# Lucaskabela/UNAST

Measured on AMD Instinct MI355X. Metric: mel-frames/sec/node (train step, gen+disc) at B=32,T_mel=800; 1/2/4/8-GPU scaling, higher is better.
Workload: dtype bf16x3

## Files before the change

include/unast_hip.h:

```cpp
#ifndef UNAST_HIP_H
#define UNAST_HIP_H
#include <stdint.h>
#ifdef __cplusplus
extern "C" {
#endif

typedef struct ihipStream_t* hipStream_t;

const char* unast_last_error(void);
int unast_version(void);
const char* unast_arch(void);

int unast_gemm(int a_mode, int b_mode, int nsplit,
               const float* A, int lda, const float* B, int ldb, float* C, int ldc,
               int M, int N, int K, int kb_valid,
               int conv_T, int conv_ca, int conv_cb, int conv_shift,
               const float* bias, const float* R, int ldr, const float* G, int ldg, float gate_scale,
               float alpha, int beta, int act,
               float drop_p, unsigned int seed, unsigned int stream_id,
               int splitk, float* splitk_ws, int64_t splitk_ws_floats, float* rowsum_a, int tile_wn, int b_presplit,
               int out_split, double* colstats, hipStream_t stream);

int unast_attn_fwd(int nsplit, const float* Q, int ldq, const float* K, int ldk, const float* V, int ldv, float* O, int ldo,
                   float* LSE, const int* lens_k, int B, int H, int Tq, int Tk, int head_dim, int causal, float scale,
                   float drop_p, unsigned int seed, unsigned int stream_id, int qkv_split, hipStream_t stream);
int unast_attn_fwd_variant(int m32);
int unast_attn_bwd(int nsplit, const float* Q, int ldq, const float* K, int ldk, const float* V, int ldv, const float* O, int ldo,
                   const float* dO, int lddo, const float* LSE, float* delta_ws, float* dQ, int lddq, float* dK, int lddk,
                   float* dV, int lddv, const int* lens_k, int B, int H, int Tq, int Tk, int head_dim, int causal, float scale,
                   float drop_p, unsigned int seed, unsigned int stream_id, int fused, int qkv_split, const int* lens_q, hipStream_t stream);

int unast_layernorm_fwd(const float* z, const float* gamma, const float* beta, float* y, float* mean, float* rstd,
                        int rows, int C, float eps, hipStream_t stream);
int unast_layernorm_bwd(const float* dy, const float* z, const float* gamma, const float* mean, const float* rstd,
                        float* dz, float* dz_drop, float* dgamma, float* dbeta, float* ws, int64_t ws_floats, int rows, int C,
                        float drop_p, unsigned int seed, unsigned int stream_id, int finalize, hipStream_t stream);
int unast_layernorm_bwd_finalize(const float* ws, int64_t ws_floats, int rows, int C, float* dgamma, float* dbeta, hipStream_t stream);
int64_t unast_layernorm_bwd_ws_floats(int rows, int C);

int unast_colsum_f32(const float* x, int ldx, int rows, int C, float* sum, hipStream_t stream);
int unast_colsum_det(const float* x, int ldx, int rows, int C, float* sum, float* ws, int64_t ws_floats, hipStream_t stream);
int64_t unast_colsum_det_ws_floats(int rows, int C);

int unast_bn_fwd(const float* x, const float* gamma, const float* beta, float* y, float* mean, float* rstd,
                 float* running_mean, float* running_var, double* ws, int rows, int C,
                 float eps, float momentum, int act, float drop_p, unsigned int seed, unsigned int stream_id,
                 int have_sums, int64_t* num_batches_tracked, hipStream_t stream);
int unast_bn_eval_fwd(const float* x, const float* gamma, const float* beta, const float* running_mean,
                      const float* running_var, float* y, float* mean, float* rstd, int rows, int C, float eps, int act,
                      hipStream_t stream);
int unast_bn_bwd(float* dy_inout, const float* x, const float* mean, const float* rstd, const float* gamma, const float* beta,
                 float* dx, float* dgamma, float* dbeta, double* ws, int rows, int C, int act,
                 float drop_p, unsigned int seed, unsigned int stream_id, int ws_zeroed, hipStream_t stream);

int unast_embed_fwd(const int64_t* ids, const float* E, float* out, int rows, int T, int D, int shift_sos,
                    float drop_p, unsigned int seed, unsigned int stream_id, float noise_p, unsigned int noise_stream,
                    hipStream_t stream);
int unast_embed_bwd(const int64_t* ids, const float* dout, float* dE, int rows, int T, int D, int vocab, int shift_sos,
                    int padding_idx, float drop_p, unsigned int seed, unsigned int stream_id, float noise_p,
                    unsigned int noise_stream, hipStream_t stream);
int unast_embed_bwd_det(const int64_t* ids, const float* dout, float* dE, int rows, int T, int D, int vocab, int shift_sos,
                        int padding_idx, float drop_p, unsigned int seed, unsigned int stream_id, float noise_p,
                        unsigned int noise_stream, hipStream_t stream);

int unast_posenc_fwd(const float* x, const float* pe, float* y, int rows, int T, int D, float scale, float drop_p,
                     unsigned int seed, unsigned int stream_id, hipStream_t stream);
int unast_posenc_bwd(const float* dy, const float* gate, float* dx, int rows, int D, float scale, float drop_p,
                     unsigned int seed, unsigned int stream_id, hipStream_t stream);

int unast_rowmask(const float* x, float* y, int rows, int D, float p, unsigned int seed, unsigned int stream_id,
                  hipStream_t stream);
int unast_add_inplace(float* a, const float* b, int64_t n, hipStream_t stream);
int unast_sum2(float* dst, const float* a, const float* b, int64_t n, hipStream_t stream);
int unast_argmax_rows(const float* x, int ld, int rows, int cols, int64_t* out, hipStream_t stream);
int unast_mask_by_len(float* x, const int64_t* lens, int B, int T, int D, hipStream_t stream);
int unast_decode_linear(const float* X, int ldx, int64_t x_pos_stride, const float* W, int ldw, const float* bias, float* Y, int ldy, int M, int N, int K,
                        int act, float drop_p, unsigned int seed, unsigned int stream_id, const float* R, int ldr,
                        int prologue, const float* ln_gamma, const float* ln_beta, float ln_eps,
                        const int64_t* tokens, int ld_tok, const float* emb, const float* pe, float pro_scale,
                        float pro_drop1, unsigned int pro_stream1, float pro_drop2, unsigned int pro_stream2,
                        float* xn_out, int ld_xn,
                        float* cache, int ld_cache, int cache_rows, int split_col, const int64_t* pos, hipStream_t stream);
int unast_decode_attn(const float* Q, int ldq, const float* K, const float* V, int ldkv, int rows_per_seq, const int* lens,
// ... 110 lines not shown
```

unast_amd/config.py:

```python
import os

NSPLIT = 1 if os.environ.get("UNAST_PREC", "bf16x3").lower() in ("bf16", "1") else 3


def set_precision(name):
    global NSPLIT
    NSPLIT = {"bf16": 1, "bf16x3": 3}[name]


def precision_name():
    return "bf16" if NSPLIT == 1 else "bf16x3"


def snapshot():
    return tuple(sorted((k, v) for k, v in globals().items() if k.isupper()))


SIDE_STREAMS = os.environ.get("UNAST_SIDE_STREAMS", "1") != "0"

DECODE_GRAPH = os.environ.get("UNAST_DECODE_GRAPH", "1") != "0"

WGRAD_STREAM_MIN_TOKENS = int(os.environ.get("UNAST_WGRAD_MIN_TOKENS", "8192"))

DETERMINISTIC_SUMS = os.environ.get("UNAST_DETERMINISTIC_SUMS", "0") == "1"

CAPTURE_PRUNE = os.environ.get("UNAST_CAPTURE_PRUNE", "1") != "0"

WGRAD_GROUP = os.environ.get("UNAST_WGRAD_GROUP", "1") != "0"

ATTN_FUSED_BWD = os.environ.get("UNAST_ATTN_FUSED_BWD", "1") != "0"
ATTN_BWD_TERMS = int(os.environ.get("UNAST_ATTN_BWD_TERMS", "3"))

DGRAD_TRANSPOSED = os.environ.get("UNAST_DGRAD_T", "0") == "1"

PANEL_MIN_ROWS = int(os.environ.get("UNAST_PANEL_MIN_ROWS", "16384"))
PANEL_ROWS = int(os.environ.get("UNAST_PANEL_ROWS", "1128"))

NATIVE_COMM = os.environ.get("UNAST_NATIVE_COMM", "1") != "0"

ENC_SKIP_PAD_GRADS = os.environ.get("UNAST_ENC_SKIP_PAD_GRADS", "0") == "1"

STREAM_JITTER = int(os.environ.get("UNAST_STREAM_JITTER", "0"))
STREAM_JITTER_SEED = int(os.environ.get("UNAST_STREAM_JITTER_SEED", "0"))

DEBUG_WORKSPACES = os.environ.get("UNAST_DEBUG_WORKSPACES", "0") == "1"

JOINT_GEN = os.environ.get("UNAST_JOINT_GEN", "1") != "0"
```

unast_amd/csrc/attention.hip:

```cpp
#include "common.h"
#include <stdlib.h>
#include <type_traits>

#define HD 64
#define ALD 64
__device__ __forceinline__ int img_off(int row, int col) { return row * (ALD * 2) + ((((col >> 3) ^ (row & 6))) << 4) + ((col & 7) << 1); }
#define LOG2E 1.4426950408889634f
#define LN2 0.6931471805599453f
#define NEG_BIG (-1.0e30f)

struct AttnParams {
    const float* Q; const float* K; const float* V; int ldq, ldk, ldv;
    float* O; int ldo;
    float* LSE;
    const float* dO; int lddo;
    const float* Delta;
    float* dK; float* dV; int lddk, lddv;
    const int* lens_k;
    const int* lens_q;
    int B, H, Tq, Tk, causal;
    float scale;
    uint32_t drop_thresh; float drop_scale; uint32_t seed, stream;
    int qkv_split;
    int order;
// ... 507 lines not shown
                    }
                }
            lsum += rs;
        };
#ifndef KO_SOFTMAX
        if (interior) softmax_tile(std::false_type{}); else softmax_tile(std::true_type{});
#endif
#pragma unroll
        for (int t2 = 0; t2 < 2; ++t2) {
            bf16x8_t vfh[2][2], vfl[2][2];
#pragma unroll
            for (int v = 0; v < 2; ++v)
#pragma unroll
                for (int dt = 0; dt < 2; ++dt) {
                    vfh[v][dt] = vtr_frag32(sV[0], 32 * t2 + 16 * v, 32 * dt, lane);
                    vfl[v][dt] = (PARTS == 2) ? vtr_frag32(sV[PARTS - 1], 32 * t2 + 16 * v, 32 * dt, lane) : vfh[v][dt];
                }
            bf16x8_t ph[2], pl[2];
#pragma unroll
            for (int v = 0; v < 2; ++v)
                split8<NSPLIT>(make_float4(s[t2][8 * v], s[t2][8 * v + 1], s[t2][8 * v + 2], s[t2][8 * v + 3]),
                               make_float4(s[t2][8 * v + 4], s[t2][8 * v + 5], s[t2][8 * v + 6], s[t2][8 * v + 7]), ph[v], pl[v]);
            asm volatile("" : "+v"(vfh[0][0]), "+v"(vfh[0][1]), "+v"(vfh[1][0]), "+v"(vfh[1][1]));
            if (PARTS == 2) asm volatile("" : "+v"(vfl[0][0]), "+v"(vfl[0][1]), "+v"(vfl[1][0]), "+v"(vfl[1][1]));
#pragma unroll
            for (int v = 0; v < 2; ++v)
#pragma unroll
                for (int dt = 0; dt < 2; ++dt) {
#ifdef KO_PVMFMA
                    o[dt][2 * t2 + v] += __builtin_bit_cast(f32x4, vfh[v][dt])[0] + __builtin_bit_cast(f32x4, vfl[v][dt])[1] + __builtin_bit_cast(f32x4, ph[v])[0] + __builtin_bit_cast(f32x4, pl[v])[1];
#else
                    o[dt] = mma3_32<NSPLIT>(vfh[v][dt], vfl[v][dt], ph[v], pl[v], o[dt]);
#endif
                }
        }
        }
#ifndef KO_BARRIER
        __syncthreads();
#endif
    }
    const float ltot = half_sum(lsum);
    if (qok) {
        const float f = ltot > 0.f ? p.drop_scale / ltot : 0.f;
        float* dst = p.O + ((size_t)b * p.Tq + q) * p.ldo + h * HD + 4 * hi;
#pragma unroll
        for (int dt = 0; dt < 2; ++dt)
#pragma unroll
            for (int i4 = 0; i4 < 4; ++i4)
                *reinterpret_cast<float4*>(dst + 32 * dt + 8 * i4) = make_float4(o[dt][4 * i4] * f, o[dt][4 * i4 + 1] * f, o[dt][4 * i4 + 2] * f, o[dt][4 * i4 + 3] * f);
        if (hi == 0) p.LSE[((size_t)b * p.H + h) * p.Tq + q] = (m + log2f(ltot)) * LN2;
    }
}

template <int NSPLIT, int FUSE_DQ, int PLO>
__global__ __launch_bounds__(256, 2) void attn_dkv_kernel(const AttnParams p) {
    constexpr int PARTS = (NSPLIT == 3) ? 2 : 1;
    constexpr int SPARTS = PLO ? PARTS : 1;
    constexpr int IMG = 32 * ALD * 2;
    constexpr int IMG128 = 128 * ALD * 2;
    __shared__ __attribute__((aligned(16))) unsigned char smem[2 * PARTS * IMG + (FUSE_DQ ? (PARTS + SPARTS) * IMG128 : 0)];
    unsigned char* sQ[2] = {smem, smem + (PARTS - 1) * IMG};
    unsigned char* sD[2] = {smem + PARTS * IMG, smem + PARTS * IMG + (PARTS - 1) * IMG};
    unsigned char* const fbase = smem + 2 * PARTS * IMG;
    unsigned char* sKs[2] = {fbase, fbase + (PARTS - 1) * IMG128};
    unsigned char* sS[2] = {fbase + PARTS * IMG128, fbase + PARTS * IMG128 + (SPARTS - 1) * IMG128};

    const int t = threadIdx.x, lane = t & 63, wave = t >> 6, l15 = lane & 15, g = lane >> 4;
    int bx, bh;
    if (!xcd_remap((p.Tk + 127) / 128, p.B * p.H, bx, bh, p.order)) return;
    const int h = bh % p.H, b = bh / p.H;
    const int kblk = bx * 128;
    const int k0 = kblk + wave * 32;
    const int klen = p.lens_k ? min(p.Tk, p.lens_k[b]) : p.Tk;
    const bool wave_live = __builtin_amdgcn_readfirstlane((int)(k0 < klen)) != 0;
    const int kk_live = min(4, (max(klen - kblk, 0) + 31) >> 5);
    const float sc = p.scale * LOG2E;
    const float* Qb = p.Q + (size_t)b * p.Tq * p.ldq + h * HD;
    const float* Kb = p.K + (size_t)b * p.Tk * p.ldk + h * HD;
    const float* Vb = p.V + (size_t)b * p.Tk * p.ldv + h * HD;
    const float* dOb = p.dO + (size_t)b * p.Tq * p.lddo + h * HD;
    const float* lseb = p.LSE + ((size_t)b * p.H + h) * p.Tq;
    const float* delb = p.Delta + ((size_t)b * p.H + h) * p.Tq;

    const bool split_in = p.qkv_split != 0;
    bf16x8_t kf[2][2][PARTS], vf[2][2][PARTS];
#pragma unroll
    for (int ks = 0; ks < 2; ++ks) {
        const int key = k0 + 16 * ks + l15;
        const bool ok = key < p.Tk;
#pragma unroll
        for (int kst = 0; kst < 2; ++kst) {
            bf16x8_t hi, lo;
            if (!FUSE_DQ) {
                load_frag8<NSPLIT>(Kb + (size_t)key * p.ldk + 32 * kst + 8 * g, ok, split_in, 1.f, hi, lo);
                kf[ks][kst][0] = hi; if (PARTS == 2) kf[ks][kst][PARTS - 1] = lo;
            }
            load_frag8<NSPLIT>(Vb + (size_t)key * p.ldv + 32 * kst + 8 * g, ok, split_in, 1.f, hi, lo);
            vf[ks][kst][0] = hi; if (PARTS == 2) vf[ks][kst][PARTS - 1] = lo;
        }
    }
    f32x4 dk[4][2], dv[4][2];
#pragma unroll
    for (int dt = 0; dt < 4; ++dt)
#pragma unroll
        for (int ks = 0; ks < 2; ++ks) { dk[dt][ks] = (f32x4){0.f, 0.f, 0.f, 0.f}; dv[dt][ks] = dk[dt][ks]; }

    const uint32_t rbase = rng_stream_base(p.seed, p.stream);
    const bool block_live = kblk < klen;
    const int qt_begin = p.causal ? (kblk / 32) : 0;
    const int qlen = p.lens_q ? min(p.Tq, max(p.lens_q[b], 0)) : p.Tq;
    const int qt_end = block_live ? (qlen + 31) / 32 : qt_begin;
    float4 rq[2], rd[2];
    float rl = 0.f, rl_cur = 0.f;
    const float* const stat_src = (lane < 32) ? lseb : delb;
    const float stat_mul = (lane < 32) ? LOG2E : 1.f;
    auto stat_load = [&](int qtile) {
        rl = stat_src[min(qtile * 32 + (lane & 31), p.Tq - 1)];
    };
    if (FUSE_DQ && qt_begin < qt_end) {
        float4 rk8[8];
        tile_load<128>(Kb + (size_t)kblk * p.ldk, p.ldk, min(128, p.Tk - kblk), rk8, t);
        tile_store<128, NSPLIT>(rk8, sKs[0], sKs[PARTS - 1], t, split_in);
    }
    if (qt_begin < qt_end) {
        tile_load<32>(Qb + (size_t)qt_begin * 32 * p.ldq, p.ldq, min(32, p.Tq - qt_begin * 32), rq, t);
        tile_load<32>(dOb + (size_t)qt_begin * 32 * p.lddo, p.lddo, min(32, p.Tq - qt_begin * 32), rd, t);
        stat_load(qt_begin);
    }
    auto dq_phase = [&](int qtile, int buf) {
        f32x4 dq[2] = {(f32x4){0.f, 0.f, 0.f, 0.f}, (f32x4){0.f, 0.f, 0.f, 0.f}};
#pragma unroll
        for (int kk = 0; kk < 4; ++kk) {
            if (kk >= kk_live) break;
            const bf16x8_t bh = tr_frag(sKs[0], 32 * kk, 16 * wave, l15, g);
            const bf16x8_t bl = (PARTS == 2) ? tr_frag(sKs[PARTS - 1], 32 * kk, 16 * wave, l15, g) : bh;
#pragma unroll
            for (int qs = 0; qs < 2; ++qs) {
                const bf16x8_t ah = tr_frag(sS[0], 32 * kk, 32 * buf + 16 * qs, l15, g);
                if (SPARTS == 2) {
                    const bf16x8_t al = tr_frag(sS[SPARTS - 1], 32 * kk, 32 * buf + 16 * qs, l15, g);
                    dq[qs] = mma3<NSPLIT>(ah, al, bh, bl, dq[qs]);
                } else {
                    dq[qs] = mma2_a<NSPLIT>(ah, bh, bl, dq[qs]);
                }
            }
        }
        float* dqb = p.O + (size_t)b * p.Tq * p.ldo + h * HD + 16 * wave + l15;
#pragma unroll
        for (int qs = 0; qs < 2; ++qs)
#pragma unroll
            for (int r = 0; r < 4; ++r) {
                const int q = qtile * 32 + 16 * qs + 4 * g + r;
                if (q < p.Tq) unsafeAtomicAdd(dqb + (size_t)q * p.ldo, dq[qs][r] * p.scale);
            }
    };
    for (int qt = qt_begin; qt < qt_end; ++qt) {
        tile_store<32, NSPLIT>(rq, sQ[0], sQ[PARTS - 1], t, split_in);
        tile_store<32, NSPLIT>(rd, sD[0], sD[PARTS - 1], t, split_in);
        rl_cur = rl * stat_mul;
        const uint32_t rk_cur = p.drop_thresh ? pcg_hash((uint32_t)(((size_t)b * p.H + h) * p.Tq + qt * 32 + (lane & 31)) + rbase) : 0u;
        __syncthreads();
        if (FUSE_DQ && qt > qt_begin) dq_phase(qt - 1, (qt - 1) & 1);
        if (qt + 1 < qt_end) {
            const int qr = (qt + 1) * 32;
            tile_load<32>(Qb + (size_t)qr * p.ldq, p.ldq, min(32, p.Tq - qr), rq, t);
            tile_load<32>(dOb + (size_t)qr * p.lddo, p.lddo, min(32, p.Tq - qr), rd, t);
            stat_load(qt + 1);
        }
        if (wave_live) {
        f32x4 s[2][2], dp[2][2];
#pragma unroll
        for (int qs = 0; qs < 2; ++qs)
#pragma unroll
            for (int ks = 0; ks < 2; ++ks) { s[qs][ks] = (f32x4){0.f, 0.f, 0.f, 0.f}; dp[qs][ks] = s[qs][ks]; }
#pragma unroll
        for (int qs = 0; qs < 2; ++qs)
#pragma unroll
            for (int kst = 0; kst < 2; ++kst) {
                const bf16x8_t qh = row_frag(sQ[0], 16 * qs, kst, l15, g);
                const bf16x8_t ql = (PARTS == 2) ? row_frag(sQ[PARTS - 1], 16 * qs, kst, l15, g) : qh;
                const bf16x8_t dh = row_frag(sD[0], 16 * qs, kst, l15, g);
                const bf16x8_t dl = (PARTS == 2) ? row_frag(sD[PARTS - 1], 16 * qs, kst, l15, g) : dh;
#pragma unroll
                for (int ks = 0; ks < 2; ++ks) {
                    if (FUSE_DQ) {
                        const bf16x8_t kh = row_frag(sKs[0], wave * 32 + 16 * ks, kst, l15, g);
                        const bf16x8_t kl = (PARTS == 2) ? row_frag(sKs[PARTS - 1], wave * 32 + 16 * ks, kst, l15, g) : kh;
                        s[qs][ks] = mma3<NSPLIT>(qh, ql, kh, kl, s[qs][ks]);
                    } else {
                        s[qs][ks] = mma3<NSPLIT>(qh, ql, kf[ks][kst][0], kf[ks][kst][PARTS - 1], s[qs][ks]);
                    }
                    dp[qs][ks] = mma3<NSPLIT>(dh, dl, vf[ks][kst][0], vf[ks][kst][PARTS - 1], dp[qs][ks]);
                }
            }
        const bool interior = (qt * 32 + 32 <= p.Tq) && (k0 + 32 <= klen) && (!p.causal || k0 + 31 <= qt * 32);
        auto pointwise = [&](auto masked_tag) {
            constexpr bool MASKED = decltype(masked_tag)::value;
            const int par = l15 & 1;
            const uint32_t sh16 = par ? 0u : 16u, thr_hi = p.drop_thresh << 16;
#pragma unroll
            for (int qs = 0; qs < 2; ++qs) {
                float l2[4], de[4];
#pragma unroll
                for (int r = 0; r < 4; ++r) {
                    l2[r] = __shfl(rl_cur, 16 * qs + 4 * g + r, 64);
                    de[r] = __shfl(rl_cur, 32 + 16 * qs + 4 * g + r, 64);
                }
                uint32_t rkm[2] = {0u, 0u};
                if (p.drop_thresh) {
#pragma unroll
                    for (int j = 0; j < 2; ++j) rkm[j] = (uint32_t)__shfl((int)rk_cur, 16 * qs + 4 * g + 2 * par + j, 64);
                }
#pragma unroll
                for (int ks = 0; ks < 2; ++ks) {
                    const int key = k0 + 16 * ks + l15;
                    uint32_t hh[4] = {0u, 0u, 0u, 0u};
                    if (p.drop_thresh) {
#pragma unroll
                        for (int j = 0; j < 2; ++j) {
                            const uint32_t hm = rng_pair(rkm[j], (uint32_t)key);
                            hh[j] = (uint32_t)__builtin_amdgcn_mov_dpp((int)hm, 0xA0, 0xF, 0xF, true);
// ... 11 lines not shown
                        float pd = pv, dpe = dp[qs][ks][r];
                        if (p.drop_thresh) {
                            const bool keep = (hh[r] << sh16) >= thr_hi;
                            pd = keep ? pv : 0.f;
                            dpe = keep ? dpe : 0.f;
                        }
                        s[qs][ks][r] = pd;
                        dp[qs][ks][r] = pv * __builtin_fmaf(dpe, p.drop_scale, -de[r]);
                    }
                }
            }
        };
        if (interior) pointwise(std::false_type{}); else pointwise(std::true_type{});
        bf16x8_t pf[2][SPARTS], sf[2][SPARTS];
#pragma unroll
        for (int ks = 0; ks < 2; ++ks) {
            bf16x8_t hi, lo;
            pack_acc<(SPARTS == 2 ? NSPLIT : 1)>(s[0][ks], s[1][ks], hi, lo);
            pf[ks][0] = hi; if (SPARTS == 2) pf[ks][SPARTS - 1] = lo;
            pack_acc<(SPARTS == 2 ? NSPLIT : 1)>(dp[0][ks], dp[1][ks], hi, lo);
            sf[ks][0] = hi; if (SPARTS == 2) sf[ks][SPARTS - 1] = lo;
            if (FUSE_DQ) {
                const int row = wave * 32 + 16 * ks + l15, col = 32 * (qt & 1) + 4 * g;
                const u32x4 hw = __builtin_bit_cast(u32x4, hi), lw = __builtin_bit_cast(u32x4, lo);
                *reinterpret_cast<u32x2*>(sS[0] + img_off(row, col)) = (u32x2){hw[0], hw[1]};
                *reinterpret_cast<u32x2*>(sS[0] + img_off(row, col + 16)) = (u32x2){hw[2], hw[3]};
                if (SPARTS == 2) {
                    *reinterpret_cast<u32x2*>(sS[SPARTS - 1] + img_off(row, col)) = (u32x2){lw[0], lw[1]};
                    *reinterpret_cast<u32x2*>(sS[SPARTS - 1] + img_off(row, col + 16)) = (u32x2){lw[2], lw[3]};
                }
            }
        }
#pragma unroll
        for (int dt = 0; dt < 4; ++dt) {
            const bf16x8_t doh = tr_frag(sD[0], 0, 16 * dt, l15, g);
            const bf16x8_t dol = (PARTS == 2) ? tr_frag(sD[PARTS - 1], 0, 16 * dt, l15, g) : doh;
            const bf16x8_t qh = tr_frag(sQ[0], 0, 16 * dt, l15, g);
            const bf16x8_t ql = (PARTS == 2) ? tr_frag(sQ[PARTS - 1], 0, 16 * dt, l15, g) : qh;
#pragma unroll
            for (int ks = 0; ks < 2; ++ks) {
                if (SPARTS == 2) {
                    dv[dt][ks] = mma3<NSPLIT>(doh, dol, pf[ks][0], pf[ks][SPARTS - 1], dv[dt][ks]);
                    dk[dt][ks] = mma3<NSPLIT>(qh, ql, sf[ks][0], sf[ks][SPARTS - 1], dk[dt][ks]);
                } else {
                    dv[dt][ks] = mma2_b<NSPLIT>(doh, dol, pf[ks][0], dv[dt][ks]);
                    dk[dt][ks] = mma2_b<NSPLIT>(qh, ql, sf[ks][0], dk[dt][ks]);
                }
            }
        }
        }
        __syncthreads();
    }
    if (FUSE_DQ && qt_begin < qt_end) dq_phase(qt_end - 1, (qt_end - 1) & 1);
#pragma unroll
    for (int ks = 0; ks < 2; ++ks) {
        const int key = k0 + 16 * ks + l15;
        if (key >= p.Tk) continue;
        float* dkp = p.dK + ((size_t)b * p.Tk + key) * p.lddk + h * HD + 4 * g;
        float* dvp = p.dV + ((size_t)b * p.Tk + key) * p.lddv + h * HD + 4 * g;
#pragma unroll
        for (int dt = 0; dt < 4; ++dt) {
            *reinterpret_cast<float4*>(dkp + 16 * dt) = make_float4(dk[dt][ks][0] * p.scale, dk[dt][ks][1] * p.scale, dk[dt][ks][2] * p.scale, dk[dt][ks][3] * p.scale);
            *reinterpret_cast<float4*>(dvp + 16 * dt) = make_float4(dv[dt][ks][0] * p.drop_scale, dv[dt][ks][1] * p.drop_scale, dv[dt][ks][2] * p.drop_scale, dv[dt][ks][3] * p.drop_scale);
        }
    }
}

__global__ __launch_bounds__(256) void attn_delta_kernel(const float* __restrict__ dO, int lddo, const float* __restrict__ O, int ldo,
                                                         float* __restrict__ delta, int rows, int Tq, int H, float* __restrict__ zero_dq, int lddq,
                                                         int do_split) {
    const int lane = threadIdx.x & 63;
    const int row = blockIdx.x * 4 + (threadIdx.x >> 6);
    if (row >= rows) return;
    const int b = row / Tq, q = row - b * Tq;
    for (int h0 = 0; h0 < H; h0 += 4) {
        const int h = h0 + (lane >> 4);
        float s = 0.f;
        if (h < H) {
            const int c = h * HD + (lane & 15) * 4;
            float4 a = *reinterpret_cast<const float4*>(dO + (size_t)row * lddo + c);
            if (do_split) {
                const uint32_t h0 = __float_as_uint(a.x), h1 = __float_as_uint(a.y), l0 = __float_as_uint(a.z), l1 = __float_as_uint(a.w);
                a.x = __uint_as_float(h0 << 16) + __uint_as_float(l0 << 16);
                a.y = __uint_as_float(h0 & 0xFFFF0000u) + __uint_as_float(l0 & 0xFFFF0000u);
                a.z = __uint_as_float(h1 << 16) + __uint_as_float(l1 << 16);
                a.w = __uint_as_float(h1 & 0xFFFF0000u) + __uint_as_float(l1 & 0xFFFF0000u);
            }
            float4 o = *reinterpret_cast<const float4*>(O + (size_t)row * ldo + c);
            s = (a.x * o.x + a.y * o.y) + (a.z * o.z + a.w * o.w);
            if (zero_dq) *reinterpret_cast<float4*>(zero_dq + (size_t)row * lddq + c) = make_float4(0.f, 0.f, 0.f, 0.f);
        }
        s += __shfl_xor(s, 1, 64); s += __shfl_xor(s, 2, 64); s += __shfl_xor(s, 4, 64); s += __shfl_xor(s, 8, 64);
        if (h < H && (lane & 15) == 0) delta[((size_t)b * H + h) * Tq + q] = s;
    }
}

static bool al16(const void* p) { return (((uintptr_t)p) & 15) == 0; }

static int fill_common(AttnParams& p, const float* Q, int ldq, const float* K, int ldk, const float* V, int ldv, const int* lens_k,
                       int B, int H, int Tq, int Tk, int head_dim, int causal, float scale, float drop_p, unsigned seed, unsigned stream_id, int qkv_split) {
    UNAST_REQUIRE(Q && K && V, "unast_attn: null Q/K/V");
    UNAST_REQUIRE(head_dim == HD, "unast_attn: this build supports head_dim=%d only (got %d)", HD, head_dim);
    UNAST_REQUIRE(B > 0 && H > 0 && Tq > 0 && Tk > 0, "unast_attn: bad dims");
    UNAST_REQUIRE(al16(Q) && al16(K) && al16(V) && (ldq & 3) == 0 && (ldk & 3) == 0 && (ldv & 3) == 0, "unast_attn: Q/K/V must be 16-byte aligned with ld%%4==0");
    UNAST_REQUIRE(!causal || Tq == Tk, "unast_attn: causal masking requires Tq == Tk");
    p.Q = Q; p.K = K; p.V = V; p.ldq = ldq; p.ldk = ldk; p.ldv = ldv; p.lens_k = lens_k;
    p.B = B; p.H = H; p.Tq = Tq; p.Tk = Tk; p.causal = causal; p.scale = scale;
    p.drop_thresh = drop_threshold(drop_p); p.drop_scale = drop_p > 0.f ? 1.f / (1.f - drop_p) : 1.f; p.seed = seed; p.stream = stream_id;
    p.qkv_split = qkv_split;
    static const int forced = [] { const char* e = getenv("UNAST_ATTN_ORDER"); return e ? atoi(e) : -1; }();
    p.order = forced >= 0 ? forced : (causal ? 1 : 0);
    p.lens_q = nullptr;
    p.O = nullptr; p.LSE = nullptr; p.dO = nullptr; p.Delta = nullptr; p.dK = nullptr; p.dV = nullptr; p.ldo = p.lddo = p.lddk = p.lddv = 0;
    return UNAST_OK;
}

static int g_attn_fwd_m32 = [] { const char* e = getenv("UNAST_ATTN_FWD_M32"); return (e && e[0] == '0') ? 0 : 1; }();
extern "C" int unast_attn_fwd_variant(int m32) {
    const int old = g_attn_fwd_m32;
    if (m32 >= 0) g_attn_fwd_m32 = m32 ? 1 : 0;
    return old;
}

extern "C" int unast_attn_fwd(int nsplit, const float* Q, int ldq, const float* K, int ldk, const float* V, int ldv, float* O, int ldo,
                              float* LSE, const int* lens_k, int B, int H, int Tq, int Tk, int head_dim, int causal, float scale,
                              float drop_p, unsigned int seed, unsigned int stream_id, int qkv_split, hipStream_t stream) {
    AttnParams p;
    int rc = fill_common(p, Q, ldq, K, ldk, V, ldv, lens_k, B, H, Tq, Tk, head_dim, causal, scale, drop_p, seed, stream_id, qkv_split);
    if (rc) return rc;
    UNAST_REQUIRE(O && LSE && al16(O) && (ldo & 3) == 0, "unast_attn_fwd: bad output");
    UNAST_REQUIRE(nsplit == 1 || nsplit == 3, "unast_attn_fwd: nsplit must be 1 or 3");
    p.O = O; p.ldo = ldo; p.LSE = LSE;
    static const bool q16 = [] { const char* e = getenv("UNAST_ATTN_FWD_Q16"); return e && e[0] == '1'; }();
    dim3 grid(xcd_grid((Tq + 127) / 128, B * H));
    if (g_attn_fwd_m32 && !q16) {
        if (nsplit == 3) hipLaunchKernelGGL((attn_fwd32_kernel<3>), grid, dim3(256), 0, stream, p);
        else             hipLaunchKernelGGL((attn_fwd32_kernel<1>), grid, dim3(256), 0, stream, p);
        return unast_check_launch("unast_attn_fwd");
    }
    if (nsplit == 3) if (q16) hipLaunchKernelGGL((attn_q_kernel<3, 0, 1>), grid, dim3(512), 0, stream, p); else hipLaunchKernelGGL((attn_q_kernel<3, 0, 2>), grid, dim3(256), 0, stream, p);
    else             if (q16) hipLaunchKernelGGL((attn_q_kernel<1, 0, 1>), grid, dim3(512), 0, stream, p); else hipLaunchKernelGGL((attn_q_kernel<1, 0, 2>), grid, dim3(256), 0, stream, p);
    return unast_check_launch("unast_attn_fwd");
}

extern "C" int unast_attn_bwd(int nsplit, const float* Q, int ldq, const float* K, int ldk, const float* V, int ldv, const float* O, int ldo,
                              const float* dO, int lddo, const float* LSE, float* delta_ws, float* dQ, int lddq, float* dK, int lddk,
                              float* dV, int lddv, const int* lens_k, int B, int H, int Tq, int Tk, int head_dim, int causal, float scale,
                              float drop_p, unsigned int seed, unsigned int stream_id, int fused, int qkv_split, const int* lens_q, hipStream_t stream) {
    AttnParams p;
    int rc = fill_common(p, Q, ldq, K, ldk, V, ldv, lens_k, B, H, Tq, Tk, head_dim, causal, scale, drop_p, seed, stream_id, qkv_split);
    if (rc) return rc;
    UNAST_REQUIRE(O && dO && LSE && delta_ws && dQ && dK && dV, "unast_attn_bwd: null pointer");
    UNAST_REQUIRE(!lens_q || fused, "unast_attn_bwd: lens_q is served by the one-pass backward (fused = 1)");
    p.lens_q = lens_q;
    UNAST_REQUIRE(al16(O) && al16(dO) && al16(dQ) && al16(dK) && al16(dV) && ((ldo | lddo | lddq | lddk | lddv) & 3) == 0,
                  "unast_attn_bwd: operands must be 16-byte aligned with ld%%4==0");
    UNAST_REQUIRE(nsplit == 1 || nsplit == 3, "unast_attn_bwd: nsplit must be 1 or 3");
    const int rows = B * Tq;
    hipLaunchKernelGGL(attn_delta_kernel, dim3((rows + 3) / 4), dim3(256), 0, stream, dO, lddo, O, ldo, delta_ws, rows, Tq, H, fused ? dQ : nullptr, lddq, qkv_split);
    p.dO = dO; p.lddo = lddo; p.LSE = const_cast<float*>(LSE); p.Delta = delta_ws;
    p.O = dQ; p.ldo = lddq; p.dK = dK; p.dV = dV; p.lddk = lddk; p.lddv = lddv;
    dim3 gq(xcd_grid((Tq + 127) / 128, B * H)), gk(xcd_grid((Tk + 127) / 128, B * H));
    if (fused) {
        if (nsplit == 3) { if (fused == 1) hipLaunchKernelGGL((attn_dkv_kernel<3, 1, 1>), gk, dim3(256), 0, stream, p); else hipLaunchKernelGGL((attn_dkv_kernel<3, 1, 0>), gk, dim3(256), 0, stream, p); }
        else             hipLaunchKernelGGL((attn_dkv_kernel<1, 1, 1>), gk, dim3(256), 0, stream, p);
    } else if (nsplit == 3) {
        hipLaunchKernelGGL((attn_q_kernel<3, 1, 2>), gq, dim3(256), 0, stream, p);
        hipLaunchKernelGGL((attn_dkv_kernel<3, 0, 1>), gk, dim3(256), 0, stream, p);
    } else {
        hipLaunchKernelGGL((attn_q_kernel<1, 1, 2>), gq, dim3(256), 0, stream, p);
        hipLaunchKernelGGL((attn_dkv_kernel<1, 0, 1>), gk, dim3(256), 0, stream, p);
    }
    return unast_check_launch("unast_attn_bwd");
}

UNAST_DEFINE_RNG_EPOCH_SETTER(attention)
```

unast_amd/ops.py:

```python
import os as _os

import torch

from . import config
from ._lib import lib, check

OP_KC, OP_KC_CONV, OP_RC, OP_RC_CONV_DGRAD, OP_RC_CONV_WGRAD = 0, 1, 2, 3, 4


def _p(t):
    return None if t is None else t.data_ptr()


_raw_stream = getattr(torch._C, "_cuda_getCurrentRawStream", None)


def _stream():
    if _raw_stream is not None:
        return _raw_stream(torch.cuda.current_device())
    return torch.cuda.current_stream().cuda_stream


_F32 = torch.float32
_LN_WS = {}


def deterministic_sums():
    return bool(config.DETERMINISTIC_SUMS)


def _f32(t, name):
    if t is None:
        return
    if not (t.is_cuda and t.dtype == torch.float32):
        raise TypeError("%s must be a float32 CUDA tensor (got %s on %s)" % (name, t.dtype, t.device))


_WEIGHT_SPANS = []


def register_weight_span(base_ptr, nbytes, split_ptr, transposed_lookup=None, planes_lookup=None):
    _WEIGHT_SPANS[:] = [s for s in _WEIGHT_SPANS if s[0] != base_ptr]
    _WEIGHT_SPANS.append((base_ptr, nbytes, split_ptr, transposed_lookup, planes_lookup))


def unregister_weight_span(base_ptr):
    _WEIGHT_SPANS[:] = [s for s in _WEIGHT_SPANS if s[0] != base_ptr]


def _weight_planes(W, transposed=False):
    ptr = W.data_ptr()
    for base, nbytes, split, _, lookup in _WEIGHT_SPANS:
        if lookup is not None and base <= ptr < base + nbytes:
            return lookup(W, transposed)
    return None


# ... 321 lines not shown
    if _PANEL_TRACE:
        print("panel_gemm M=%d N=%d K=%d lda=%d ldc=%d bias=%s R=%s G=%s act=%d drop=%.2f split=%d ln=%s bits=%s rows=%d" % (
            M, N, K, A.stride(0), C.stride(0), bias is not None, R is not None, G is not None, act, drop_p, out_split, ln is not None,
            None if gate_bits is None else gate_bits.numel(), rows_per_wg), flush=True)
    check(lib().unast_panel_gemm(_p(A), A.stride(0), wplanes[0], wplanes[1], _p(C), C.stride(0), M, N, K, _p(bias), _p(R),
                                 R.stride(0) if R is not None else 0, _p(G), G.stride(0) if G is not None else 0, gate_scale, act,
                                 drop_p, seed & 0xFFFFFFFF, stream_id, int(out_split), _p(g), _p(b), _p(Y), ldy, _p(mean), _p(rstd), eps,
                                 _p(gate_bits), rows_per_wg, _stream()), "unast_panel_gemm")
    if _PANEL_TRACE:
        torch.cuda.synchronize()
    return C


def conv_fwd(x3d, Wp, bias, out, pad_left, colstats=None):
    B, T, Cin = x3d.shape
    Cout = Wp.shape[0]
    gemm(OP_KC_CONV, OP_KC, x3d, x3d.stride(1), Wp, 5 * Cin, out, out.stride(1), B * T, Cout, 5 * Cin,
         conv=(T, Cin, 0, pad_left), bias=bias, colstats=colstats)
    return out


def conv_dgrad(dy3d, Wp, dx, pad_left, beta=0):
    B, T, Cout = dy3d.shape
    Cin = Wp.shape[2]
    gemm(OP_KC_CONV, OP_RC_CONV_DGRAD, dy3d, dy3d.stride(1), Wp, 4, dx, dx.stride(1), B * T, Cin, 5 * Cout,
         conv=(T, Cout, Cout, 4 - pad_left), beta=beta)
    return dx


def conv_wgrad(dy3d, x3d, dWp, pad_left, db=None):
    B, T, Cout = dy3d.shape
    Cin = x3d.shape[2]
    sk = _splitk_for(Cout, 5 * Cin, B * T)
    if db is not None and deterministic_sums() and dy3d.is_contiguous():
        def both():
            gemm(OP_RC, OP_RC_CONV_WGRAD, dy3d, dy3d.stride(1), x3d, x3d.stride(1), dWp, 5 * Cin, Cout, 5 * Cin, B * T,
                 conv=(T, 0, Cin, pad_left), beta=1, splitk=sk)
            colsum(dy3d.view(B * T, Cout), db)
        _on_wgrad_stream(both, B * T, dWp.data_ptr(), dy3d, x3d)
        return dWp
    _on_wgrad_stream(lambda: gemm(OP_RC, OP_RC_CONV_WGRAD, dy3d, dy3d.stride(1), x3d, x3d.stride(1), dWp, 5 * Cin, Cout, 5 * Cin, B * T,
                                  conv=(T, 0, Cin, pad_left), beta=1, splitk=sk, rowsum_a=db), B * T, dWp.data_ptr(), dy3d, x3d)
    return dWp


def attn_fwd(Q, K, V, O, LSE, lens_k, B, H, Tq, Tk, causal, drop_p=0.0, seed=0, stream_id=0, nsplit=None, qkv_split=False):
    check(lib().unast_attn_fwd(nsplit or config.NSPLIT, _p(Q), Q.stride(0), _p(K), K.stride(0), _p(V), V.stride(0), _p(O), O.stride(0),
                               _p(LSE), _p(lens_k), B, H, Tq, Tk, 64, int(causal), 0.125, drop_p, seed & 0xFFFFFFFF, stream_id,
                               int(qkv_split), _stream()), "unast_attn_fwd")


def attn_bwd(Q, K, V, O, dO, LSE, delta_ws, dQ, dK, dV, lens_k, B, H, Tq, Tk, causal, drop_p=0.0, seed=0, stream_id=0, nsplit=None, qkv_split=False, lens_q=None):
    fused = config.ATTN_FUSED_BWD and not deterministic_sums()
    check(lib().unast_attn_bwd(nsplit or config.NSPLIT, _p(Q), Q.stride(0), _p(K), K.stride(0), _p(V), V.stride(0), _p(O), O.stride(0),
                               _p(dO), dO.stride(0), _p(LSE), _p(delta_ws), _p(dQ), dQ.stride(0), _p(dK), dK.stride(0), _p(dV),
                               dV.stride(0), _p(lens_k), B, H, Tq, Tk, 64, int(causal), 0.125, drop_p, seed & 0xFFFFFFFF, stream_id,
                               (2 if config.ATTN_BWD_TERMS == 2 else 1) if fused else 0, int(qkv_split),
                               _p(lens_q) if fused else None, _stream()), "unast_attn_bwd")


def layernorm_fwd(z, gamma, beta, y, mean, rstd, eps=1e-5):
    rows, C = z.shape
    check(lib().unast_layernorm_fwd(_p(z), _p(gamma), _p(beta), _p(y), _p(mean), _p(rstd), rows, C, eps, _stream()), "unast_layernorm_fwd")


def layernorm_bwd(dy, z, gamma, mean, rstd, dz, dz_drop=None, dgamma=None, dbeta=None, drop_p=0.0, seed=0, stream_id=0):
    rows, C = z.shape
    ws, ws_n = None, 0
    if dgamma is not None:
        ws_n = _LN_WS.get((rows, C))
        if ws_n is None:
            ws_n = _LN_WS[(rows, C)] = lib().unast_layernorm_bwd_ws_floats(rows, C)
        ws = torch.empty(ws_n, dtype=torch.float32, device=z.device)
    check(lib().unast_layernorm_bwd(_p(dy), _p(z), _p(gamma), _p(mean), _p(rstd), _p(dz), _p(dz_drop), _p(dgamma), _p(dbeta), _p(ws), ws_n,
                                    rows, C, drop_p, seed & 0xFFFFFFFF, stream_id, 0 if dgamma is not None else 1, _stream()), "unast_layernorm_bwd")
    if dgamma is not None:
        _on_wgrad_stream(lambda: check(lib().unast_layernorm_bwd_finalize(_p(ws), ws_n, rows, C, _p(dgamma), _p(dbeta), _stream()),
                                       "unast_layernorm_bwd_finalize"), rows, dgamma.data_ptr(), ws)


def colsum(x2d, out):
    rows, C = x2d.shape
    if deterministic_sums():
        ws_n = lib().unast_colsum_det_ws_floats(rows, C)
        ws = torch.empty(ws_n, dtype=torch.float32, device=x2d.device)
        check(lib().unast_colsum_det(_p(x2d), x2d.stride(0), rows, C, _p(out), _p(ws), ws_n, _stream()), "unast_colsum_det")
        return
    check(lib().unast_colsum_f32(_p(x2d), x2d.stride(0), rows, C, _p(out), _stream()), "unast_colsum_f32")


def bn_fwd(x2d, gamma, beta, y, mean, rstd, running_mean, running_var, ws, act, drop_p=0.0, seed=0, stream_id=0, eps=1e-5, momentum=0.1, have_sums=False,
           num_batches_tracked=None):
    rows, C = x2d.shape
    check(lib().unast_bn_fwd(_p(x2d), _p(gamma), _p(beta), _p(y), _p(mean), _p(rstd), _p(running_mean), _p(running_var), _p(ws), rows, C,
                             eps, momentum, act, drop_p, seed & 0xFFFFFFFF, stream_id, int(have_sums), _p(num_batches_tracked), _stream()), "unast_bn_fwd")


def bn_eval_fwd(x2d, gamma, beta, running_mean, running_var, y, mean, rstd, act, eps=1e-5):
    rows, C = x2d.shape
    check(lib().unast_bn_eval_fwd(_p(x2d), _p(gamma), _p(beta), _p(running_mean), _p(running_var), _p(y), _p(mean), _p(rstd), rows, C,
                                  eps, act, _stream()), "unast_bn_eval_fwd")


def bn_bwd(dy_inout, x2d, mean, rstd, gamma, beta, dx, dgamma, dbeta, ws, act, drop_p=0.0, seed=0, stream_id=0, ws_zeroed=False):
    rows, C = x2d.shape
    check(lib().unast_bn_bwd(_p(dy_inout), _p(x2d), _p(mean), _p(rstd), _p(gamma), _p(beta), _p(dx), _p(dgamma), _p(dbeta), _p(ws), rows, C,
                             act, drop_p, seed & 0xFFFFFFFF, stream_id, int(ws_zeroed), _stream()), "unast_bn_bwd")


def embed_fwd(ids, E, out, T, shift_sos=-1, drop_p=0.0, seed=0, stream_id=0, noise_p=0.0, noise_stream=0):
    rows = ids.numel()
# ... 346 lines not shown
```

Measured before the change: 944,900.

## Add wide 8-wave attention dK/dV kernel with plain dQ stores for short keys

```diff
diff --git a/include/unast_hip.h b/include/unast_hip.h
--- a/include/unast_hip.h
+++ b/include/unast_hip.h
@@ -28,7 +28,7 @@
 int unast_attn_bwd(int nsplit, const float* Q, int ldq, const float* K, int ldk, const float* V, int ldv, const float* O, int ldo,
                    const float* dO, int lddo, const float* LSE, float* delta_ws, float* dQ, int lddq, float* dK, int lddk,
                    float* dV, int lddv, const int* lens_k, int B, int H, int Tq, int Tk, int head_dim, int causal, float scale,
-                   float drop_p, unsigned int seed, unsigned int stream_id, int fused, int qkv_split, const int* lens_q, hipStream_t stream);
+                   float drop_p, unsigned int seed, unsigned int stream_id, int fused, int qkv_split, const int* lens_q, int form, hipStream_t stream);
 
 int unast_layernorm_fwd(const float* z, const float* gamma, const float* beta, float* y, float* mean, float* rstd,
                         int rows, int C, float eps, hipStream_t stream);
diff --git a/unast_amd/attn_form.py b/unast_amd/attn_form.py
--- /dev/null
+++ b/unast_amd/attn_form.py
@@ -0,0 +1,38 @@
+from . import config
+
+NARROW, WIDE, STORE = 0, 1, 2
+NAMES = {NARROW: "narrow", WIDE: "wide", STORE: "store"}
+KEYS = {NARROW: 128, WIDE: 256, STORE: 256}
+CUS = 256
+ATOMIC_BYTES_PER_S = 1.3e12
+
+
+def key_blocks(form, Tk):
+    return -(-Tk // KEYS[form])
+
+
+def workgroups(form, B, H, Tk):
+    return key_blocks(form, Tk) * B * H
+
+
+def atomic_bytes(form, B, H, Tq, Tk, causal):
+    if form == STORE:
+        return 0
+    kb = KEYS[form]
+    rows = sum((Tq - min(i * kb, Tq)) if causal else Tq for i in range(key_blocks(form, Tk)))
+    return B * H * rows * 64 * 4
+
+
+def atomic_floor_us(form, B, H, Tq, Tk, causal):
+    return atomic_bytes(form, B, H, Tq, Tk, causal) / ATOMIC_BYTES_PER_S * 1e6
+
+
+def choose(B, H, Tq, Tk, causal=False):
+    forced = config.ATTN_BWD_FORM
+    if forced not in ("auto", "narrow", "wide"):
+        raise ValueError("config.ATTN_BWD_FORM must be 'auto', 'narrow' or 'wide' (got %r)" % (forced,))
+    if forced == "narrow":
+        return NARROW
+    if Tk <= KEYS[STORE]:
+        return STORE
+    return WIDE if forced == "wide" or workgroups(WIDE, B, H, Tk) >= CUS else NARROW
diff --git a/unast_amd/config.py b/unast_amd/config.py
--- a/unast_amd/config.py
+++ b/unast_amd/config.py
@@ -30,6 +30,7 @@
 
 ATTN_FUSED_BWD = os.environ.get("UNAST_ATTN_FUSED_BWD", "1") != "0"
 ATTN_BWD_TERMS = int(os.environ.get("UNAST_ATTN_BWD_TERMS", "3"))
+ATTN_BWD_FORM = os.environ.get("UNAST_ATTN_BWD_FORM", "auto")
 
 DGRAD_TRANSPOSED = os.environ.get("UNAST_DGRAD_T", "0") == "1"
 
diff --git a/unast_amd/csrc/attention.hip b/unast_amd/csrc/attention.hip
--- a/unast_amd/csrc/attention.hip
+++ b/unast_amd/csrc/attention.hip
@@ -583,28 +583,30 @@
     }
 }
 
-template <int NSPLIT, int FUSE_DQ, int PLO>
-__global__ __launch_bounds__(256, 2) void attn_dkv_kernel(const AttnParams p) {
+template <int NSPLIT, int FUSE_DQ, int PLO, int NW = 4, int DQ_STORE = 0>
+__global__ __launch_bounds__(64 * NW, 2) void attn_dkv_kernel(const AttnParams p) {
+    static_assert(NW == 4 || NW == 8, "4 or 8 waves");
+    constexpr int NT = 64 * NW, KB = 32 * NW;
     constexpr int PARTS = (NSPLIT == 3) ? 2 : 1;
     constexpr int SPARTS = PLO ? PARTS : 1;
     constexpr int IMG = 32 * ALD * 2;
-    constexpr int IMG128 = 128 * ALD * 2;
-    __shared__ __attribute__((aligned(16))) unsigned char smem[2 * PARTS * IMG + (FUSE_DQ ? (PARTS + SPARTS) * IMG128 : 0)];
+    constexpr int IMGK = KB * ALD * 2;
+    __shared__ __attribute__((aligned(16))) unsigned char smem[2 * PARTS * IMG + (FUSE_DQ ? (PARTS + SPARTS) * IMGK : 0)];
     unsigned char* sQ[2] = {smem, smem + (PARTS - 1) * IMG};
     unsigned char* sD[2] = {smem + PARTS * IMG, smem + PARTS * IMG + (PARTS - 1) * IMG};
     unsigned char* const fbase = smem + 2 * PARTS * IMG;
-    unsigned char* sKs[2] = {fbase, fbase + (PARTS - 1) * IMG128};
-    unsigned char* sS[2] = {fbase + PARTS * IMG128, fbase + PARTS * IMG128 + (SPARTS - 1) * IMG128};
+    unsigned char* sKs[2] = {fbase, fbase + (PARTS - 1) * IMGK};
+    unsigned char* sS[2] = {fbase + PARTS * IMGK, fbase + PARTS * IMGK + (SPARTS - 1) * IMGK};
 
     const int t = threadIdx.x, lane = t & 63, wave = t >> 6, l15 = lane & 15, g = lane >> 4;
     int bx, bh;
-    if (!xcd_remap((p.Tk + 127) / 128, p.B * p.H, bx, bh, p.order)) return;
+    if (!xcd_remap((p.Tk + KB - 1) / KB, p.B * p.H, bx, bh, p.order)) return;
     const int h = bh % p.H, b = bh / p.H;
-    const int kblk = bx * 128;
+    const int kblk = bx * KB;
     const int k0 = kblk + wave * 32;
     const int klen = p.lens_k ? min(p.Tk, p.lens_k[b]) : p.Tk;
     const bool wave_live = __builtin_amdgcn_readfirstlane((int)(k0 < klen)) != 0;
-    const int kk_live = min(4, (max(klen - kblk, 0) + 31) >> 5);
+    const int kk_live = min(NW, (max(klen - kblk, 0) + 31) >> 5);
     const float sc = p.scale * LOG2E;
     const float* Qb = p.Q + (size_t)b * p.Tq * p.ldq + h * HD;
     const float* Kb = p.K + (size_t)b * p.Tk * p.ldk + h * HD;
@@ -641,7 +643,7 @@
     const int qt_begin = p.causal ? (kblk / 32) : 0;
     const int qlen = p.lens_q ? min(p.Tq, max(p.lens_q[b], 0)) : p.Tq;
     const int qt_end = block_live ? (qlen + 31) / 32 : qt_begin;
-    float4 rq[2], rd[2];
+    float4 rq[32 * 16 / NT], rd[32 * 16 / NT];
     float rl = 0.f, rl_cur = 0.f;
     const float* const stat_src = (lane < 32) ? lseb : delb;
     const float stat_mul = (lane < 32) ? LOG2E : 1.f;
@@ -650,54 +652,62 @@
     };
     if (FUSE_DQ && qt_begin < qt_end) {
         float4 rk8[8];
-        tile_load<128>(Kb + (size_t)kblk * p.ldk, p.ldk, min(128, p.Tk - kblk), rk8, t);
-        tile_store<128, NSPLIT>(rk8, sKs[0], sKs[PARTS - 1], t, split_in);
+        tile_load<KB, NT>(Kb + (size_t)kblk * p.ldk, p.ldk, min(KB, p.Tk - kblk), rk8, t);
+        tile_store<KB, NSPLIT, NT>(rk8, sKs[0], sKs[PARTS - 1], t, split_in);
     }
     if (qt_begin < qt_end) {
-        tile_load<32>(Qb + (size_t)qt_begin * 32 * p.ldq, p.ldq, min(32, p.Tq - qt_begin * 32), rq, t);
-        tile_load<32>(dOb + (size_t)qt_begin * 32 * p.lddo, p.lddo, min(32, p.Tq - qt_begin * 32), rd, t);
+        tile_load<32, NT>(Qb + (size_t)qt_begin * 32 * p.ldq, p.ldq, min(32, p.Tq - qt_begin * 32), rq, t);
+        tile_load<32, NT>(dOb + (size_t)qt_begin * 32 * p.lddo, p.lddo, min(32, p.Tq - qt_begin * 32), rd, t);
         stat_load(qt_begin);
     }
+    constexpr int NQS = 8 / NW;
+    const int dq_d0 = 16 * (wave & 3), dq_qs0 = (NW == 8) ? (wave >> 2) : 0;
     auto dq_phase = [&](int qtile, int buf) {
-        f32x4 dq[2] = {(f32x4){0.f, 0.f, 0.f, 0.f}, (f32x4){0.f, 0.f, 0.f, 0.f}};
-#pragma unroll
-        for (int kk = 0; kk < 4; ++kk) {
+        f32x4 dq[NQS];
+#pragma unroll
+        for (int qi = 0; qi < NQS; ++qi) dq[qi] = (f32x4){0.f, 0.f, 0.f, 0.f};
+#pragma unroll
+        for (int kk = 0; kk < NW; ++kk) {
             if (kk >= kk_live) break;
-            const bf16x8_t bh = tr_frag(sKs[0], 32 * kk, 16 * wave, l15, g);
-            const bf16x8_t bl = (PARTS == 2) ? tr_frag(sKs[PARTS - 1], 32 * kk, 16 * wave, l15, g) : bh;
-#pragma unroll
-            for (int qs = 0; qs < 2; ++qs) {
-                const bf16x8_t ah = tr_frag(sS[0], 32 * kk, 32 * buf + 16 * qs, l15, g);
+            const bf16x8_t bh = tr_frag(sKs[0], 32 * kk, dq_d0, l15, g);
+            const bf16x8_t bl = (PARTS == 2) ? tr_frag(sKs[PARTS - 1], 32 * kk, dq_d0, l15, g) : bh;
+#pragma unroll
+            for (int qi = 0; qi < NQS; ++qi) {
+                const int qcol = 32 * buf + 16 * (dq_qs0 + qi);
+                const bf16x8_t ah = tr_frag(sS[0], 32 * kk, qcol, l15, g);
                 if (SPARTS == 2) {
-                    const bf16x8_t al = tr_frag(sS[SPARTS - 1], 32 * kk, 32 * buf + 16 * qs, l15, g);
-                    dq[qs] = mma3<NSPLIT>(ah, al, bh, bl, dq[qs]);
+                    const bf16x8_t al = tr_frag(sS[SPARTS - 1], 32 * kk, qcol, l15, g);
+                    dq[qi] = mma3<NSPLIT>(ah, al, bh, bl, dq[qi]);
                 } else {
-                    dq[qs] = mma2_a<NSPLIT>(ah, bh, bl, dq[qs]);
-                }
-            }
-        }
-        float* dqb = p.O + (size_t)b * p.Tq * p.ldo + h * HD + 16 * wave + l15;
-#pragma unroll
-        for (int qs = 0; qs < 2; ++qs)
+                    dq[qi] = mma2_a<NSPLIT>(ah, bh, bl, dq[qi]);
+                }
+            }
+        }
+        float* dqb = p.O + (size_t)b * p.Tq * p.ldo + h * HD + dq_d0 + l15;
+#pragma unroll
+        for (int qi = 0; qi < NQS; ++qi)
 #pragma unroll
             for (int r = 0; r < 4; ++r) {
-                const int q = qtile * 32 + 16 * qs + 4 * g + r;
-                if (q < p.Tq) unsafeAtomicAdd(dqb + (size_t)q * p.ldo, dq[qs][r] * p.scale);
+                const int q = qtile * 32 + 16 * (dq_qs0 + qi) + 4 * g + r;
+                if (q < p.Tq) {
+                    if (DQ_STORE) dqb[(size_t)q * p.ldo] = dq[qi][r] * p.scale;
+                    else unsafeAtomicAdd(dqb + (size_t)q * p.ldo, dq[qi][r] * p.scale);
+                }
             }
     };
     for (int qt = qt_begin; qt < qt_end; ++qt) {
-        tile_store<32, NSPLIT>(rq, sQ[0], sQ[PARTS - 1], t, split_in);
-        tile_store<32, NSPLIT>(rd, sD[0], sD[PARTS - 1], t, split_in);
+        tile_store<32, NSPLIT, NT>(rq, sQ[0], sQ[PARTS - 1], t, split_in);
+        tile_store<32, NSPLIT, NT>(rd, sD[0], sD[PARTS - 1], t, split_in);
         rl_cur = rl * stat_mul;
         const uint32_t rk_cur = p.drop_thresh ? pcg_hash((uint32_t)(((size_t)b * p.H + h) * p.Tq + qt * 32 + (lane & 31)) + rbase) : 0u;
         __syncthreads();
-        if (FUSE_DQ && qt > qt_begin) dq_phase(qt - 1, (qt - 1) & 1);
         if (qt + 1 < qt_end) {
             const int qr = (qt + 1) * 32;
-            tile_load<32>(Qb + (size_t)qr * p.ldq, p.ldq, min(32, p.Tq - qr), rq, t);
-            tile_load<32>(dOb + (size_t)qr * p.lddo, p.lddo, min(32, p.Tq - qr), rd, t);
+            tile_load<32, NT>(Qb + (size_t)qr * p.ldq, p.ldq, min(32, p.Tq - qr), rq, t);
+            tile_load<32, NT>(dOb + (size_t)qr * p.lddo, p.lddo, min(32, p.Tq - qr), rd, t);
             stat_load(qt + 1);
         }
+        if (FUSE_DQ && qt > qt_begin) dq_phase(qt - 1, (qt - 1) & 1);
         if (wave_live) {
         f32x4 s[2][2], dp[2][2];
 #pragma unroll
@@ -815,6 +825,10 @@
         __syncthreads();
     }
     if (FUSE_DQ && qt_begin < qt_end) dq_phase(qt_end - 1, (qt_end - 1) & 1);
+    if (FUSE_DQ && DQ_STORE) {
+        for (int idx = qt_end * 32 * 16 + t; idx < p.Tq * 16; idx += NT)
+            *reinterpret_cast<float4*>(p.O + ((size_t)b * p.Tq + (idx >> 4)) * p.ldo + h * HD + (idx & 15) * 4) = make_float4(0.f, 0.f, 0.f, 0.f);
+    }
 #pragma unroll
     for (int ks = 0; ks < 2; ++ks) {
         const int key = k0 + 16 * ks + l15;
@@ -909,7 +923,7 @@
 extern "C" int unast_attn_bwd(int nsplit, const float* Q, int ldq, const float* K, int ldk, const float* V, int ldv, const float* O, int ldo,
                               const float* dO, int lddo, const float* LSE, float* delta_ws, float* dQ, int lddq, float* dK, int lddk,
                               float* dV, int lddv, const int* lens_k, int B, int H, int Tq, int Tk, int head_dim, int causal, float scale,
-                              float drop_p, unsigned int seed, unsigned int stream_id, int fused, int qkv_split, const int* lens_q, hipStream_t stream) {
+                              float drop_p, unsigned int seed, unsigned int stream_id, int fused, int qkv_split, const int* lens_q, int form, hipStream_t stream) {
     AttnParams p;
     int rc = fill_common(p, Q, ldq, K, ldk, V, ldv, lens_k, B, H, Tq, Tk, head_dim, causal, scale, drop_p, seed, stream_id, qkv_split);
     if (rc) return rc;
@@ -919,12 +933,21 @@
     UNAST_REQUIRE(al16(O) && al16(dO) && al16(dQ) && al16(dK) && al16(dV) && ((ldo | lddo | lddq | lddk | lddv) & 3) == 0,
                   "unast_attn_bwd: operands must be 16-byte aligned with ld%%4==0");
     UNAST_REQUIRE(nsplit == 1 || nsplit == 3, "unast_attn_bwd: nsplit must be 1 or 3");
+    UNAST_REQUIRE(form >= 0 && form <= 2, "unast_attn_bwd: form must be 0, 1 or 2 (got %d)", form);
+    UNAST_REQUIRE(!fused || form != 2 || Tk <= 256, "unast_attn_bwd: form 2 (plain dQ stores) serves one key block, Tk <= 256 (got %d)", Tk);
+    const bool dq_store = fused && form == 2;
     const int rows = B * Tq;
-    hipLaunchKernelGGL(attn_delta_kernel, dim3((rows + 3) / 4), dim3(256), 0, stream, dO, lddo, O, ldo, delta_ws, rows, Tq, H, fused ? dQ : nullptr, lddq, qkv_split);
+    hipLaunchKernelGGL(attn_delta_kernel, dim3((rows + 3) / 4), dim3(256), 0, stream, dO, lddo, O, ldo, delta_ws, rows, Tq, H, (fused && !dq_store) ? dQ : nullptr, lddq, qkv_split);
     p.dO = dO; p.lddo = lddo; p.LSE = const_cast<float*>(LSE); p.Delta = delta_ws;
     p.O = dQ; p.ldo = lddq; p.dK = dK; p.dV = dV; p.lddk = lddk; p.lddv = lddv;
-    dim3 gq(xcd_grid((Tq + 127) / 128, B * H)), gk(xcd_grid((Tk + 127) / 128, B * H));
-    if (fused) {
+    dim3 gq(xcd_grid((Tq + 127) / 128, B * H)), gk(xcd_grid((Tk + 127) / 128, B * H)), gk8(xcd_grid((Tk + 255) / 256, B * H));
+    if (dq_store) {
+        if (nsplit == 3) { if (fused == 1) hipLaunchKernelGGL((attn_dkv_kernel<3, 1, 1, 8, 1>), gk8, dim3(512), 0, stream, p); else hipLaunchKernelGGL((attn_dkv_kernel<3, 1, 0, 8, 1>), gk8, dim3(512), 0, stream, p); }
+        else             hipLaunchKernelGGL((attn_dkv_kernel<1, 1, 1, 8, 1>), gk8, dim3(512), 0, stream, p);
+    } else if (fused && form == 1) {
+        if (nsplit == 3) { if (fused == 1) hipLaunchKernelGGL((attn_dkv_kernel<3, 1, 1, 8>), gk8, dim3(512), 0, stream, p); else hipLaunchKernelGGL((attn_dkv_kernel<3, 1, 0, 8>), gk8, dim3(512), 0, stream, p); }
+        else             hipLaunchKernelGGL((attn_dkv_kernel<1, 1, 1, 8>), gk8, dim3(512), 0, stream, p);
+    } else if (fused) {
         if (nsplit == 3) { if (fused == 1) hipLaunchKernelGGL((attn_dkv_kernel<3, 1, 1>), gk, dim3(256), 0, stream, p); else hipLaunchKernelGGL((attn_dkv_kernel<3, 1, 0>), gk, dim3(256), 0, stream, p); }
         else             hipLaunchKernelGGL((attn_dkv_kernel<1, 1, 1>), gk, dim3(256), 0, stream, p);
     } else if (nsplit == 3) {
diff --git a/unast_amd/ops.py b/unast_amd/ops.py
--- a/unast_amd/ops.py
+++ b/unast_amd/ops.py
@@ -2,7 +2,7 @@
 
 import torch
 
-from . import config
+from . import attn_form, config
 from ._lib import lib, check
 
 OP_KC, OP_KC_CONV, OP_RC, OP_RC_CONV_DGRAD, OP_RC_CONV_WGRAD = 0, 1, 2, 3, 4
@@ -430,11 +430,13 @@
 
 def attn_bwd(Q, K, V, O, dO, LSE, delta_ws, dQ, dK, dV, lens_k, B, H, Tq, Tk, causal, drop_p=0.0, seed=0, stream_id=0, nsplit=None, qkv_split=False, lens_q=None):
     fused = config.ATTN_FUSED_BWD and not deterministic_sums()
+    form = attn_form.choose(B, H, Tq, Tk, causal) if fused else attn_form.NARROW
     check(lib().unast_attn_bwd(nsplit or config.NSPLIT, _p(Q), Q.stride(0), _p(K), K.stride(0), _p(V), V.stride(0), _p(O), O.stride(0),
                                _p(dO), dO.stride(0), _p(LSE), _p(delta_ws), _p(dQ), dQ.stride(0), _p(dK), dK.stride(0), _p(dV),
                                dV.stride(0), _p(lens_k), B, H, Tq, Tk, 64, int(causal), 0.125, drop_p, seed & 0xFFFFFFFF, stream_id,
                                (2 if config.ATTN_BWD_TERMS == 2 else 1) if fused else 0, int(qkv_split),
-                               _p(lens_q) if fused else None, _stream()), "unast_attn_bwd")
+                               _p(lens_q) if fused else None, form, _stream()), "unast_attn_bwd")
+    return form if fused else None
 
 
 def layernorm_fwd(z, gamma, beta, y, mean, rstd, eps=1e-5):
```

Measured after the change: 931,100. 0.985x the previous value.
